# leonsick/s2d

Hardware: AMD Instinct MI355X
Metric: clip-frames/sec fwd+loss, R50 M2F-Video T=8 720p Q=100 (higher is better)
Workload: dtype f32 (f16x3 MFMA for dense contractions); 1 GPU; KDVideoMaskFormer fwd+loss (student+teacher fwd, GT+KD VideoSetCriterion), c4: 2 clips/GPU x T=8 x 720x1280, Q=100, P=160000, N=10 sparse GT instances/clip, encoder dropout 0.3; clips_per_gpu=2, frames_per_clip=8, parallelism=dp1 (clips sharded, no collective), streams=2

## Files before the change

include/s2d_hip.h:

```cpp
#ifndef S2D_HIP_H
#define S2D_HIP_H
#include <stdint.h>

#ifndef HIP_INCLUDE_HIP_HIP_RUNTIME_API_H
typedef struct ihipStream_t *hipStream_t;
#endif

#ifdef __cplusplus
extern "C" {
#endif

#define S2D_OK 0
#define S2D_ERR_ARG (-1)
#define S2D_ERR_LAUNCH (-2)

int s2d_abi_version(void);

int s2d_set_dense_mode(int mode);


int s2d_gemm_nt_f32(const float *A, const float *B, float *C, int M, int N, int K, long lda, long ldb, long ldc,
                    int batch, long strideA, long strideB, long strideC, const float *scale, const float *bias,
                    const float *res, long ldr, long strideR, int res_rows, int res_cols, int relu, const void *B_split,
                    hipStream_t stream);
// ... 6 lines not shown

int s2d_gemm_nt_gate_f32(const float *A, const float *B, float *C, int M, int N, int K, long lda, long ldb, long ldc, const float *scale,
                         const float *res, long ldr, const float *gate, long ldg, float gate_scale, const void *B_split, hipStream_t stream);
int s2d_conv2d_nhwc_gate_f32(const float *x, const float *w, float *y, int N, int H, int W, int Cin, int Cout, int KH, int KW, int stride,
                             int pad, const float *scale, const float *gate, float gate_scale, const void *w_split, hipStream_t stream);
int s2d_gemm_nt_presplit_f32(const void *A_split, const float *B, float *C, int M, int N, int K, long ldb, long ldc, const float *bias,
                             const float *res, long ldr, int res_rows, int res_cols, int relu, const void *B_split, hipStream_t stream);
long s2d_split_weights_words(int N, int K);
long s2d_gemm_rows_launches(void);
int s2d_split_weights_f16(const float *W, int N, int K, long ldw, void *out, hipStream_t stream);

long s2d_ffn_pack_words(int C, int F, int Npost, int pre);
int s2d_ffn_pack_f16(const float *W1, const float *W2, int C, int F, const float *Wpost, int Npost, const float *Wpre, void *out,
                     hipStream_t stream);
int s2d_ffn_fused_f32(const float *x, long M, int C, int F, const void *pack, const float *b1, const float *b2, const float *ln1_gamma,
                      const float *ln1_beta, const float *ln2_gamma, const float *ln2_beta, float eps, float p, uint64_t seed,
                      unsigned site_hidden, unsigned site_out, unsigned row0, float *xn, float *y, int Npost, const float *post_bias,
                      const float *post_pos, int post_S, int post_npos, long post_ldpos, float *post_out, long post_ld,
                      const float *pre_bias, const float *pre_res, unsigned site_pre, hipStream_t stream);

int s2d_conv2d_nhwc_f32(const float *x, const float *w, float *y, int N, int H, int W, int Cin, int Cout, int KH,
                        int KW, int stride, int pad, const float *scale, const float *bias, const float *res,
                        int relu, const void *w_split, hipStream_t stream);

int s2d_gemm_nt_amp_f32(const float *A, const float *B, float *C, int M, int N, int K, long lda, long ldb, long ldc, int batch,
                        long strideA, long strideB, long strideC, const float *scale, const float *bias, const float *res, long ldr,
                        long strideR, int res_rows, int res_cols, int relu, hipStream_t stream);
int s2d_conv2d_nhwc_amp_f32(const float *x, const float *w, float *y, int N, int H, int W, int Cin, int Cout, int KH, int KW, int stride,
                            int pad, const float *scale, const float *bias, const float *res, int relu, hipStream_t stream);


int s2d_msda_forward_f32(const float *value, const int64_t *shapes_host, const int64_t *level_start_host,
                         const float *loc, const float *attn_w, int N, int S, int M, int D, int L, int Lq, int P,
                         float *out, hipStream_t stream);

int s2d_msda_backward_f32(const float *value, const int64_t *shapes_host, const int64_t *level_start_host,
                          const float *loc, const float *attn_w, const float *grad_out, int N, int S, int M, int D,
                          int L, int Lq, int P, float *grad_value, float *grad_loc, float *grad_attn_w,
                          hipStream_t stream);

long s2d_msda_backward_workspace_bytes(const int64_t *shapes_host, int N, int M, int L, int Lq, int P);
int s2d_msda_backward_sorted_f32(const float *value, const int64_t *shapes_host, const int64_t *level_start_host,
                                 const float *loc, const float *attn_w, const float *grad_out, int N, int S, int M, int D,
                                 int L, int Lq, int P, float *grad_value, float *grad_loc, float *grad_attn_w, void *workspace,
                                 long workspace_bytes, hipStream_t stream);
int s2d_msda_backward_sorted_strided_f32(const float *value, long ldv, const int64_t *shapes_host, const int64_t *level_start_host,
// ... 424 lines not shown
```

s2d_amd/csrc/gemm.hip:

```cpp
#include "gemm_epilogue.h"
#include "dropout.h"

namespace {

constexpr int BM = 128, BN = 128, BK = 32, LDS_STRIDE = BK + 4;

template <bool CONV>
__global__ __launch_bounds__(256, 2) void gemm_nt_kernel(GemmParams p)
{
    __shared__ __attribute__((aligned(16))) float lds[2 * (BM + BN) * LDS_STRIDE];
    float *As = lds;
    float *Bs = lds + 2 * BM * LDS_STRIDE;

    const int tid = threadIdx.x, lane = tid & 63, wave = tid >> 6;
    const int wm = wave >> 1, wn = wave & 1;
    const int l32 = lane & 31, h = lane >> 5;

    const int tiles_n = (p.N + BN - 1) / BN, tiles_m = (p.M + BM - 1) / BM;
    const int nwg = tiles_m * tiles_n;
    int bid = blockIdx.x;
    {
        const int q = nwg / 8, r = nwg % 8, xcd = bid % 8, within = bid / 8;
        bid = (xcd < r ? xcd * (q + 1) : r * (q + 1) + (xcd - r) * q) + within;
    }
// ... 205 lines not shown
    q.drop_thresh = thresh;
    q.drop_scale = s2d_dropout_scale(thresh);
    q.drop_k0 = (unsigned)(seed & 0xFFFFFFFFull); q.drop_k1 = (unsigned)(seed >> 32); q.drop_stream = site; q.drop_row0 = row0;
    return launch(q, false, 1, stream);
}

int s2d_conv2d_nhwc_f32(const float *x, const float *w, float *y, int N, int H, int W, int Cin, int Cout, int KH,
                        int KW, int stride, int pad, const float *scale, const float *bias, const float *res,
                        int relu, const void *w_split, hipStream_t stream)
{
    if (Cin & 3) return S2D_ERR_ARG;
    GemmParams p{};
    p.Bsplit = reinterpret_cast<const unsigned int *>(w_split);
    p.Hin = H; p.Win = W; p.Cin = Cin; p.KH = KH; p.KW = KW; p.stride = stride; p.pad = pad;
    p.Hout = (H + 2 * pad - KH) / stride + 1;
    p.Wout = (W + 2 * pad - KW) / stride + 1;
    p.A = x; p.B = w; p.C = y;
    p.M = N * p.Hout * p.Wout; p.N = Cout; p.K = KH * KW * Cin;
    p.lda = 4; p.ldb = p.K; p.ldc = Cout;
    p.scale = scale; p.bias = bias; p.res = res; p.ldr = Cout; p.relu = relu; p.res_cols = Cout;
    return launch(p, true, 1, stream);
}

int s2d_conv2d_nhwc_gate_f32(const float *x, const float *w, float *y, int N, int H, int W, int Cin, int Cout, int KH, int KW, int stride,
                             int pad, const float *scale, const float *gate, float gate_scale, const void *w_split, hipStream_t stream)
{
    if ((Cin & 3) || !gate) return S2D_ERR_ARG;
    GemmParams p{};
    p.Bsplit = reinterpret_cast<const unsigned int *>(w_split);
    p.Hin = H; p.Win = W; p.Cin = Cin; p.KH = KH; p.KW = KW; p.stride = stride; p.pad = pad;
    p.Hout = (H + 2 * pad - KH) / stride + 1;
    p.Wout = (W + 2 * pad - KW) / stride + 1;
    p.A = x; p.B = w; p.C = y;
    p.M = N * p.Hout * p.Wout; p.N = Cout; p.K = KH * KW * Cin;
    p.lda = 4; p.ldb = p.K; p.ldc = Cout;
    p.scale = scale; p.ldr = Cout; p.res_cols = Cout;
    p.gate = gate; p.ldg = Cout; p.gate_scale = gate_scale;
    return launch(p, true, 1, stream);
}

}

extern "C" long s2d_split_weights_words(int N, int K) { return (long)N * ((K + 31) / 32) * 32; }

extern "C" int s2d_split_weights_f16(const float *W, int N, int K, long ldw, void *out, hipStream_t stream)
{
    if (N < 0 || K <= 0 || ldw < K) return S2D_ERR_ARG;
    return s2d_split_weights_launch(W, N, K, ldw, reinterpret_cast<unsigned int *>(out), stream, g_dense_mode == 1);
}

extern "C" int s2d_abi_version(void) { return 11; }

extern "C" int s2d_set_dense_mode(int mode)
{
    if (mode < 0 || mode > 2) return S2D_ERR_ARG;
    g_dense_mode = mode;
    return S2D_OK;
}
```

s2d_amd/csrc/gemm_bf16.hip:

```cpp
#include "gemm_epilogue.h"
#include "gemm_route.h"
#include "dropout.h"
#include <type_traits>

namespace {

typedef __bf16 bf16x2 __attribute__((ext_vector_type(2)));
typedef __bf16 bf16x8 __attribute__((ext_vector_type(8)));

constexpr int BN = GEMM_BN, BK = GEMM_BK, ROWW = 36;

__device__ __forceinline__ void split4_bf16(const f32x4 v, u32x2 &hi, u32x2 &lo)
{
    const f32x2 a = {v[0], v[1]}, b = {v[2], v[3]};
    const bf16x2 ha = __builtin_convertvector(a, bf16x2), hb = __builtin_convertvector(b, bf16x2);
    const unsigned int ua = __builtin_bit_cast(unsigned int, ha), ub = __builtin_bit_cast(unsigned int, hb);
    const f32x2 fa = {__uint_as_float(ua << 16), __uint_as_float(ua & 0xFFFF0000u)};
    const f32x2 fb = {__uint_as_float(ub << 16), __uint_as_float(ub & 0xFFFF0000u)};
    const bf16x2 la = __builtin_convertvector(a - fa, bf16x2), lb = __builtin_convertvector(b - fb, bf16x2);
    hi[0] = ua; hi[1] = ub;
    lo[0] = __builtin_bit_cast(unsigned int, la); lo[1] = __builtin_bit_cast(unsigned int, lb);
}

template <int WM, bool CONV>
// ... 701 lines not shown
            }
        }
        return;
    }
#pragma unroll
    for (int tn = 0; tn < 2; ++tn) {
        const int col = n0 + wn * 64 + tn * 32 + l32;
        if (col >= p.N) continue;
        const float sc = p.scale ? p.scale[col] : 1.f;
        const float bi = p.bias ? p.bias[col] : 0.f;
#pragma unroll
        for (int tm = 0; tm < 2; ++tm) {
#pragma unroll
            for (int r = 0; r < 16; ++r) {
                const int row = mfma32_row(r, h, m0 + wm * 64 + tm * 32);
                if (row >= p.M) continue;
                C[(long)row * p.ldc + col] = scalar_tail(p, res, join(accm[tm][tn][r], accx[tm][tn][r]), sc, bi, row, col);
            }
        }
    }
}

constexpr int HT_H = HALO_PH, HT_W = HALO_PW, HALO_W = HT_W + 2;
template <int PH, int WNW, bool PIPE>
__global__ __launch_bounds__(256, 2) void conv3x3_f16x3_halo_kernel(GemmParams p)
{
    constexpr int HALO_ROWS = (PH + 2) * HALO_W, BNT = 64 * WNW, WROWS = BNT / 32;
    static_assert(PH * HT_W == 64 * (4 / WNW), "four waves of 64 pixels x 64 channels");
    extern __shared__ __attribute__((aligned(16))) unsigned int lds[];
    unsigned int *Ah = lds;
    unsigned int *Bs = lds + HALO_ROWS * ROWW;
    const int tid = threadIdx.x, lane = tid & 63, wave = tid >> 6;
    const int wm = wave / WNW, wn = wave % WNW;
    const int l32 = lane & 31, h = lane >> 5;
    const int H = p.Hin, W = p.Win, Cin = p.Cin;
    const int tiles_x = (W + HT_W - 1) / HT_W, tiles_y = (H + PH - 1) / PH;
    const int tiles_n = (p.N + BNT - 1) / BNT, tiles_m = (p.M / (H * W)) * tiles_y * tiles_x;
    const int nwg = tiles_m * tiles_n;
    int bid = blockIdx.x;
    {
        const int q = nwg / 8, r = nwg % 8, xcd = bid % 8, within = bid / 8;
        bid = (xcd < r ? xcd * (q + 1) : r * (q + 1) + (xcd - r) * q) + within;
    }
    const int tile_m = bid / tiles_n, tile_n = bid % tiles_n;
    const int n0 = tile_n * BNT;
    const int img = tile_m / (tiles_y * tiles_x), trem = tile_m % (tiles_y * tiles_x);
    const int y0 = (trem / tiles_x) * PH, x0 = (trem % tiles_x) * HT_W;

    const __amdgpu_buffer_rsrc_t rsA = __builtin_amdgcn_make_buffer_rsrc(const_cast<float *>(p.A), 0, (int)p.bytesA, 0x00020000);
    const __amdgpu_buffer_rsrc_t rsB = __builtin_amdgcn_make_buffer_rsrc(const_cast<unsigned int *>(p.Bsplit), 0, (int)((long)p.N * p.kblocks * 128L), 0x00020000);
    constexpr int A_IT = (HALO_ROWS * 8 + 255) / 256;
    unsigned int ha_off[A_IT];
    int ha_dst[A_IT];
    bool ha_zero[A_IT];
#pragma unroll
    for (int i = 0; i < A_IT; ++i) {
        const int item = tid + 256 * i;
        const int row = item >> 3, c4 = item & 7;
        const int hy = row / HALO_W, hx = row - hy * HALO_W;
        const int iy = y0 - 1 + hy, ix = x0 - 1 + hx;
        const bool ok = row < HALO_ROWS && iy >= 0 && iy < H && ix >= 0 && ix < W;
        ha_off[i] = ok ? (unsigned int)((((long)img * H + iy) * W + ix) * Cin * 4L + c4 * 16) : 0u;
        ha_zero[i] = !ok;
        ha_dst[i] = row < HALO_ROWS ? row * ROWW + c4 * 2 : -1;
    }
    const int c4 = tid & 7, g = tid >> 3;
    const int r0 = (g & ~7) | ((g & 1) << 2) | ((g >> 1) & 3);
    const int wsel = (c4 & 3) * 4 + (c4 >> 2) * 16;
    unsigned int b_off[WROWS];
#pragma unroll
    for (int i = 0; i < WROWS; ++i) {
        const int n = n0 + r0 + 32 * i;
        b_off[i] = (unsigned int)((long)(n < p.N ? n : p.N - 1) * p.kblocks * 128L + wsel * 4);
    }
    const int cblocks = Cin / 32;
    f32x4 ra[A_IT], rb[WROWS];
    auto load_halo = [&](int cb) {
#pragma unroll
        for (int i = 0; i < A_IT; ++i)
            ra[i] = __builtin_bit_cast(f32x4, __builtin_amdgcn_raw_buffer_load_b128(rsA, (int)(ha_off[i] + (ha_zero[i] ? 0u : (unsigned int)(cb * 128))), 0, 0));
    };
    auto store_halo = [&]() {
#pragma unroll
        for (int i = 0; i < A_IT; ++i) {
            if (ha_dst[i] < 0) continue;
            u32x2 hi, lo;
            split4(ra[i], hi, lo);
            if (ha_zero[i]) { hi = u32x2{0u, 0u}; lo = u32x2{0u, 0u}; }
            *reinterpret_cast<u32x2 *>(Ah + ha_dst[i]) = hi;
            *reinterpret_cast<u32x2 *>(Ah + ha_dst[i] + 16) = lo;
        }
    };
    auto load_w = [&](int tap, int cb) {
        const unsigned int kb = (unsigned int)(tap * cblocks + cb) * 128u;
#pragma unroll
        for (int i = 0; i < WROWS; ++i)
            rb[i] = __builtin_bit_cast(f32x4, __builtin_amdgcn_raw_buffer_load_b128(rsB, (int)b_off[i], (int)kb, 0));
    };
    auto store_w = [&](int buf) {
#pragma unroll
        for (int i = 0; i < WROWS; ++i)
            *reinterpret_cast<f32x4 *>(Bs + (buf * BNT + r0 + 32 * i) * ROWW + wsel) = rb[i];
    };
    int a_row[2];
#pragma unroll
    for (int i = 0; i < 2; ++i) {
        const int pix = wm * 64 + i * 32 + l32;
        a_row[i] = ((pix / HT_W) * HALO_W + (pix % HT_W)) * ROWW + 4 * h;
    }
    f32x16 accm[2][2], accx[2][2];
#pragma unroll
    for (int i = 0; i < 2; ++i)
#pragma unroll
// ... 45 lines not shown
        accx[i][0] = __builtin_amdgcn_mfma_f32_32x32x16_f16(pa[bufi][0], pb[s][0][1], accx[i][0], 0, 0, 0);
        accx[i][1] = __builtin_amdgcn_mfma_f32_32x32x16_f16(pa[bufi][0], pb[s][1][1], accx[i][1], 0, 0, 0);
        accm[i][0] = __builtin_amdgcn_mfma_f32_32x32x16_f16(pa[bufi][0], pb[s][0][0], accm[i][0], 0, 0, 0);
        accm[i][1] = __builtin_amdgcn_mfma_f32_32x32x16_f16(pa[bufi][0], pb[s][1][0], accm[i][1], 0, 0, 0);
    };
    auto compute_pipe = [&](int tap, int buf, int ntap, bool nexta) {
        read_a(1, tap, 0, 1); read_b(buf, 1);
        __builtin_amdgcn_sched_barrier(0);
        group(0, 0, 0);
        __builtin_amdgcn_sched_barrier(0);
        read_a(0, tap, 1, 0);
        __builtin_amdgcn_sched_barrier(0);
        group(1, 0, 1);
        __builtin_amdgcn_sched_barrier(0);
        read_a(1, tap, 1, 1);
        __builtin_amdgcn_sched_barrier(0);
        group(0, 1, 0);
        __builtin_amdgcn_sched_barrier(0);
        if (nexta) read_a(0, ntap, 0, 0);
        __builtin_amdgcn_sched_barrier(0);
        group(1, 1, 1);
        __builtin_amdgcn_sched_barrier(0);
    };
    constexpr bool pipe = PIPE;
    load_halo(0); load_w(0, 0);
    store_halo(); store_w(0);
    __syncthreads();
    const int Q = cblocks * 9;
    int tap = 0, cb = 0;
    if (pipe) { read_a(0, 0, 0, 0); read_b(0, 0); }
    for (int q = 0; q < Q; ++q) {
        const int ntap = tap == 8 ? 0 : tap + 1, ncb = tap == 8 ? cb + 1 : cb;
        if (q + 1 < Q) load_w(ntap, ncb);
        if (tap == 6 && cb + 1 < cblocks) load_halo(cb + 1);
        const bool newhalo = tap == 8 && cb + 1 < cblocks;
        if (pipe) compute_pipe(tap, q & 1, ntap, q + 1 < Q && !newhalo);
        else compute(tap, q & 1);
        if (q + 1 < Q) store_w((q + 1) & 1);
        __syncthreads();
        if (newhalo) { store_halo(); __syncthreads(); }
        if (pipe && q + 1 < Q) {
            if (newhalo) read_a(0, ntap, 0, 0);
            read_b((q + 1) & 1, 0);
        }
        tap = ntap; cb = ncb;
    }

    float *ep = reinterpret_cast<float *>(lds) + wave * 64 * 68;
#pragma unroll
    for (int tm = 0; tm < 2; ++tm)
#pragma unroll
        for (int tn = 0; tn < 2; ++tn)
#pragma unroll
            for (int r = 0; r < 16; ++r)
                ep[mfma32_row(r, h, tm * 32) * 68 + tn * 32 + l32] = join(accm[tm][tn][r], accx[tm][tn][r]);
    const int c4e = lane & 15, rr = lane >> 4;
    const int col = n0 + wn * 64 + c4e * 4;
    if (col < p.N) {
        f32x4 sc = {1.f, 1.f, 1.f, 1.f}, bi = {0.f, 0.f, 0.f, 0.f};
        if (p.scale) sc = *reinterpret_cast<const f32x4 *>(p.scale + col);
        if (p.bias) bi = *reinterpret_cast<const f32x4 *>(p.bias + col);
#pragma unroll 4
        for (int it = 0; it < 16; ++it) {
            const int pix = wm * 64 + it * 4 + rr;
            const int oy = y0 + pix / HT_W, ox = x0 + pix % HT_W;
            if (oy >= H || ox >= W) continue;
            const long row = ((long)img * H + oy) * W + ox;
            f32x4 v = *reinterpret_cast<const f32x4 *>(&ep[(it * 4 + rr) * 68 + c4e * 4]);
// ... 773 lines not shown

int launch_conv7x7s2_stem(const GemmParams &p, int ph, hipStream_t st)
{
    const size_t lds16 = sizeof(float) * 4 * 64 * 68, lds8 = sizeof(float) * 4 * 32 * 68;
    static S2dDevOnce attr_set;
    if (!attr_set.done()) {
        if (hipFuncSetAttribute(reinterpret_cast<const void *>(conv7x7s2_c4_halo_kernel<16>), hipFuncAttributeMaxDynamicSharedMemorySize, (int)lds16) != hipSuccess)
            return S2D_ERR_LAUNCH;
        attr_set.mark();
    }
    const int imgs = p.M / (p.Hout * p.Wout);
    if (ph == 16) hipLaunchKernelGGL(conv7x7s2_c4_halo_kernel<16>, dim3(imgs * cdiv(p.Hout, 16) * cdiv(p.Wout, ST_P)), dim3(256), lds16, st, p);
    else hipLaunchKernelGGL(conv7x7s2_c4_halo_kernel<8>, dim3(imgs * cdiv(p.Hout, 8) * cdiv(p.Wout, ST_P)), dim3(256), lds8, st, p);
    S2D_CHECK_LAUNCH();
    return S2D_OK;
}

int launch_conv3x3_halo(const GemmParams &p, const GemmRoute &r, hipStream_t st)
{
    const size_t lds = sizeof(float) * 4 * 64 * 68;
    static S2dDevOnce attr_set;
    if (!attr_set.done()) {
        for (const void *fn : {reinterpret_cast<const void *>(conv3x3_f16x3_halo_kernel<8, 2, true>), reinterpret_cast<const void *>(conv3x3_f16x3_halo_kernel<16, 1, true>),
                               reinterpret_cast<const void *>(conv3x3_f16x3_halo_kernel<8, 2, false>), reinterpret_cast<const void *>(conv3x3_f16x3_halo_kernel<16, 1, false>)})
            if (hipFuncSetAttribute(fn, hipFuncAttributeMaxDynamicSharedMemorySize, (int)lds) != hipSuccess) return S2D_ERR_LAUNCH;
        attr_set.mark();
    }
    const int imgs = p.M / (p.Hin * p.Win);
    if (r.ph == 16) {
        const int nwg = imgs * cdiv(p.Hin, 16) * cdiv(p.Win, HT_W);
        if (r.pipe) hipLaunchKernelGGL((conv3x3_f16x3_halo_kernel<16, 1, true>), dim3(nwg), dim3(256), lds, st, p);
        else hipLaunchKernelGGL((conv3x3_f16x3_halo_kernel<16, 1, false>), dim3(nwg), dim3(256), lds, st, p);
    } else {
        const int nwg = imgs * cdiv(p.Hin, HT_H) * cdiv(p.Win, HT_W) * cdiv(p.N, BN);
        if (r.pipe) hipLaunchKernelGGL((conv3x3_f16x3_halo_kernel<8, 2, true>), dim3(nwg), dim3(256), lds, st, p);
        else hipLaunchKernelGGL((conv3x3_f16x3_halo_kernel<8, 2, false>), dim3(nwg), dim3(256), lds, st, p);
    }
    S2D_CHECK_LAUNCH();
    return S2D_OK;
}

template <bool CONV, bool BSPLIT>
int launch_w128_v(const GemmParams &p, int batch, hipStream_t st)
{
    const size_t lds = sizeof(float) * 4 * 64 * 68;
    static S2dDevOnce attr_set;
    if (!attr_set.done()) {
        if (hipFuncSetAttribute(reinterpret_cast<const void *>(gemm_bf16x3_w128_kernel<CONV, BSPLIT>),
                                hipFuncAttributeMaxDynamicSharedMemorySize, (int)lds) != hipSuccess)
            return S2D_ERR_LAUNCH;
        attr_set.mark();
    }
    const int nwg = cdiv(p.M, 256) * cdiv(p.N, BN);
    hipLaunchKernelGGL((gemm_bf16x3_w128_kernel<CONV, BSPLIT>), dim3(nwg, batch), dim3(256), lds, st, p);
    S2D_CHECK_LAUNCH();
    return S2D_OK;
}

// ... 28 lines not shown
    const int k = kb * 32 + c4 * 4;
    f32x4 v = {0.f, 0.f, 0.f, 0.f};
    if (vec4) { if (k < K) v = *reinterpret_cast<const f32x4 *>(W + n * ldw + k); }
    else {
        float t[4] = {0.f, 0.f, 0.f, 0.f};
#pragma unroll
        for (int j = 0; j < 4; ++j)
            if (k + j < K) t[j] = W[n * ldw + k + j];
#pragma unroll
        for (int j = 0; j < 4; ++j) {
            float r;
            asm volatile("v_mov_b32 %0, %1" : "=v"(r) : "v"(t[j]));
            v[j] = r;
        }
    }
    u32x2 hi, lo;
    if (BF16) split4_bf16(v, hi, lo);
    else split4(v, hi, lo);
    unsigned int *o = out + nb * 32;
    *reinterpret_cast<u32x2 *>(o + c4 * 2) = hi;
    *reinterpret_cast<u32x2 *>(o + 16 + c4 * 2) = lo;
}

}

int s2d_split_weights_launch(const float *W, int N, int K, long ldw, unsigned int *out, hipStream_t st, int bf16)
{
    const int kblocks = (K + 31) / 32;
    const long n = (long)N * kblocks * 8;
    if (n == 0) return S2D_OK;
    const int vec4 = ((K | ldw) & 3) == 0 && (reinterpret_cast<uintptr_t>(W) & 15) == 0;
    if (bf16) hipLaunchKernelGGL(split_weights_kernel<true>, dim3(cdiv(n, 256)), dim3(256), 0, st, W, N, K, ldw, kblocks, out, vec4);
    else hipLaunchKernelGGL(split_weights_kernel<false>, dim3(cdiv(n, 256)), dim3(256), 0, st, W, N, K, ldw, kblocks, out, vec4);
    S2D_CHECK_LAUNCH();
    return S2D_OK;
}

static GemmSwitches read_gemm_switches()
{
    GemmSwitches s;
    static const int small = s2d_env_int("S2D_GEMM_SMALL", s.small), ws = s2d_env_int("S2D_GEMM_WS", s.ws), hi = s2d_env_int("S2D_GEMM_HI", s.hi),
                     hi_pre = s2d_env_int("S2D_GEMM_HI_PRE", s.hi_pre), pipe = s2d_env_int("S2D_GEMM_PIPE", s.pipe), w128 = s2d_env_int("S2D_GEMM_W128", s.w128),
                     wm = s2d_env_int("S2D_GEMM_WM", s.wm), halo = s2d_env_int("S2D_CONV_HALO", s.halo), halo64 = s2d_env_int("S2D_CONV_HALO64", s.halo64),
                     stem = s2d_env_int("S2D_CONV_STEM", s.stem), stem_ph = s2d_env_int("S2D_CONV_STEM_PH", s.stem_ph);
    s.small = small; s.ws = ws; s.hi = hi; s.hi_pre = hi_pre; s.pipe = pipe; s.w128 = w128; s.wm = wm; s.halo = halo; s.halo64 = halo64; s.stem = stem; s.stem_ph = stem_ph;
    s.rows = s2d_env_int("S2D_GEMM_ROWS", s.rows);
// ... 38 lines not shown
```

s2d_amd/csrc/gemm_params.h:

```cpp
#pragma once

struct GemmParams {
    const float *A, *B;
    float *C;
    int M, N, K;
    long lda, ldb, ldc;
    long sA, sB, sC;
    const float *scale, *bias, *res;
    long ldr, sR;
    int res_rows, res_cols;
    int relu;
    const float *gate;
    long ldg;
    float gate_scale;
    int Hin, Win, Cin, Hout, Wout, KH, KW, stride, pad;
    unsigned int bytesA, bytesB;
    const unsigned int *Bsplit;
    int kblocks;
    const unsigned int *Asplit;
    unsigned int drop_thresh;
    float drop_scale;
    unsigned int drop_k0, drop_k1, drop_stream;
    unsigned int drop_row0;
    const float *zeros, *ones;
};

#ifdef __HIPCC__
struct GemmSwitches;
int s2d_split_weights_launch(const float *W, int N, int K, long ldw, unsigned int *out, hipStream_t st, int bf16);
int s2d_launch_gemm_bf16x3(const GemmParams &p, bool conv, int batch, hipStream_t st, int f16);
int s2d_launch_gemm_small_m(const GemmParams &p, hipStream_t st);
int s2d_launch_gemm_rows(const GemmParams &p, const GemmSwitches &sw, hipStream_t st);
#endif
```

s2d_amd/csrc/gemm_route.h:

```cpp
#pragma once
#include <stdint.h>

#include "gemm_params.h"

constexpr int GEMM_BN = 128, GEMM_BK = 32;
constexpr int HALO_PH = 8, HALO_PW = 16;
constexpr int WS_CONST_N = 16384;

struct GemmSwitches {
    int rows = 1, small = 1, ws = 0, hi = 2, hi_pre = 1, pipe = 1, w128 = 1, wm = 0;
    int halo = 1, halo64 = 1, halo_pipe = 0, stem = 1, stem_ph = 8;
};

enum GemmFamily {
    GEMM_ERR_ARG, GEMM_ROWS, GEMM_SMALL_M, GEMM_F16_WS, GEMM_F16_HI, GEMM_F16, GEMM_CONV3X3_HALO, GEMM_CONV7X7S2_STEM, GEMM_W128, GEMM_T2, GEMM_T4
};

struct GemmRoute {
    GemmFamily family = GEMM_ERR_ARG;
    bool conv = false, bsplit = false, drop = false, res = false, asplit = false;
    bool pipe = false, pre = false;
    int ph = 0;
};

static inline int gemm_cdiv(long a, long b) { return (int)((a + b - 1) / b); }

inline bool s2d_gemm_extents(GemmParams &p, bool conv, int batch)
{
    const long bA = conv ? (long)(p.M / ((long)p.Hout * p.Wout)) * p.Hin * p.Win * p.Cin * 4L : ((long)(p.M - 1) * p.lda + p.K) * 4L;
    const long bB = ((long)(p.N - 1) * p.ldb + p.K) * 4L;
    if (bA > 0xFFFFFF00L || bB > 0xFFFFFF00L) return false;
    p.bytesA = (unsigned int)bA; p.bytesB = (unsigned int)bB;
    if (p.Bsplit) {
        if ((batch > 1 && p.sB != 0) || (long)p.N * ((p.K + 31) / 32) * 128L > 0xFFFFFF00L) return false;
        p.kblocks = (p.K + 31) / 32;
    }
    return true;
}

inline bool s2d_gemm_rows_ok(const GemmParams &p, bool conv, int batch, int f16)
{
    const long bC = ((long)(p.M - 1) * p.ldc + p.N) * 4L, bR = p.res ? ((long)((p.res_rows ? p.res_rows : p.M) - 1) * p.ldr + p.N) * 4L : 0;
    return f16 && !conv && batch == 1 && p.M >= 1 && p.Bsplit && !p.Asplit && !p.gate && !p.drop_thresh && p.K % 32 == 0 && p.K >= 32 && p.K <= 256 &&
           p.N >= 128 && ((p.N | p.ldc | p.ldr | p.res_cols) & 3) == 0 && bC <= 0xFFFFFF00L && bR <= 0xFFFFFF00L;
}

inline bool s2d_gemm_small_m_ok(const GemmParams &p, bool conv, int batch, int f16, const GemmSwitches &sw)
{
    return sw.small && f16 && !conv && batch == 1 && p.M >= 1 && p.M <= 256 && p.Bsplit && !p.Asplit && !p.gate && !p.drop_thresh && p.K >= 64 && p.K % 64 == 0 &&
           (p.lda & 3) == 0 && ((reinterpret_cast<uintptr_t>(p.A) & 15) == 0);
}

inline bool gemm_rows_wins(const GemmParams &p)
{
    if (p.M >= 65536) return (long)p.N * p.K >= 65536;
    return p.M >= 32768 && p.N >= 1024 && p.K >= 256;
}

inline GemmRoute s2d_gemm_route(const GemmParams &p, bool conv, int batch, int f16, const GemmSwitches &sw)
{
    constexpr int BN = GEMM_BN, BK = GEMM_BK;
    GemmRoute r;
    const auto to = [&r](GemmFamily f) { r.family = f; return r; };
    if (!f16 && (p.Asplit || p.gate || p.drop_thresh)) return to(GEMM_ERR_ARG);
    if (sw.rows && s2d_gemm_rows_ok(p, conv, batch, f16) && (sw.rows == 2 || gemm_rows_wins(p))) return to(GEMM_ROWS);
    if (s2d_gemm_small_m_ok(p, conv, batch, f16, sw)) return to(GEMM_SMALL_M);
    r.conv = conv; r.bsplit = p.Bsplit != nullptr; r.drop = p.drop_thresh != 0; r.res = p.res != nullptr;

    const long bC = ((long)(p.M - 1) * p.ldc + p.N) * 4L, bR = p.res ? ((long)((p.res_rows ? p.res_rows : p.M) - 1) * p.ldr + p.N) * 4L : 0;
    const bool ws_ok = sw.ws && f16 && batch == 1 && !p.gate && p.N <= WS_CONST_N && (conv || !p.scale) && p.K >= 7 * BK - (BK - 1) && ((p.N | p.ldc | p.ldr | p.res_cols) & 3) == 0 &&
                       (conv ? (p.Cin % 4 == 0 && (p.Bsplit || p.K % BK == 0)) : p.K % BK == 0) &&
                       bC <= 0xFFFFFF00L && bR <= 0xFFFFFF00L && (!p.res_rows || p.res_rows >= 64) &&
                       (!p.drop_thresh || (((p.N | p.ldc) & 7) == 0 && (!p.res || ((p.ldr | p.res_cols) & 7) == 0)));
    if (p.Asplit) {
        const bool ok = f16 && !conv && batch == 1 && p.Bsplit && !p.scale && p.N <= WS_CONST_N && p.K >= 7 * BK - (BK - 1) && p.K % BK == 0 &&
                        ((p.N | p.ldc | p.ldr | p.res_cols) & 3) == 0 && bC <= 0xFFFFFF00L && bR <= 0xFFFFFF00L &&
                        (long)p.M * p.kblocks * 128L <= 0xFFFFFF00L && (!p.res_rows || p.res_rows >= 64) &&
                        (!p.drop_thresh || (((p.N | p.ldc) & 7) == 0 && (!p.res || ((p.ldr | p.res_cols) & 7) == 0)));
        if (!ok) return to(GEMM_ERR_ARG);
        r.asplit = true;
        return to(GEMM_F16_WS);
    }
    if (ws_ok && !conv && (sw.ws == 2 || (p.Bsplit && (long)gemm_cdiv(p.M, 128) * gemm_cdiv(p.N, BN) >= 512))) return to(GEMM_F16_WS);
    if (ws_ok && conv && !p.drop_thresh && (sw.ws == 2 || (long)gemm_cdiv(p.M, 128) * gemm_cdiv(p.N, BN) >= 512)) return to(GEMM_F16_WS);
    if (p.gate && (!f16 || batch != 1 || p.drop_thresh || ((p.N | p.ldc | p.ldr | p.res_cols | p.ldg) & 3))) return to(GEMM_ERR_ARG);
    if (p.drop_thresh) {
        if (!f16 || conv || ((p.N | p.ldc) & 7) || (p.res && (((p.ldr | p.res_cols) & 7)))) return to(GEMM_ERR_ARG);
        r.pipe = true;
        return to(GEMM_F16);
    }
    if (f16) {
        if (sw.stem && conv && p.KH == 7 && p.KW == 7 && p.stride == 2 && p.pad == 3 && p.Cin == 4 && p.N <= 64 && p.N > 32 && p.Bsplit && batch == 1 &&
            ((p.N | p.ldc | p.ldr) & 3) == 0 && !p.res_rows && p.res_cols == p.N && !p.gate && (long)p.Hin * p.Win * 16L * (p.M / ((long)p.Hout * p.Wout)) < 0x7fffffffL) {
            r.ph = sw.stem_ph == 16 ? 16 : 8;
            return to(GEMM_CONV7X7S2_STEM);
        }
        const int ph = p.N <= 64 ? 16 : HALO_PH;
        if (sw.halo && conv && p.KH == 3 && p.KW == 3 && p.stride == 1 && p.pad == 1 && p.Cin % 32 == 0 && p.Bsplit && batch == 1 && (p.N > 64 || (sw.halo64 && p.N > 32)) &&
            ((p.N | p.ldc | p.ldr) & 3) == 0 && !p.res_rows && p.res_cols == p.N && !p.gate &&
            (sw.halo == 2 || (long)p.Hin * p.Win * 100 >= (long)gemm_cdiv(p.Hin, ph) * ph * gemm_cdiv(p.Win, HALO_PW) * HALO_PW * 88)) {
            r.ph = ph;
            r.pipe = sw.halo_pipe != 0;
            return to(GEMM_CONV3X3_HALO);
        }
        bool use_hi;
        if (sw.hi != 2) use_hi = sw.hi == 1;
        else if (conv && p.KH > 1) use_hi = p.N <= 64;
        else if (p.N <= 64 || p.K <= 128 || !p.Bsplit) use_hi = true;
        else if (p.K >= 512) use_hi = false;
        else {
            const float w128 = (float)(gemm_cdiv(p.N, 128) * 128) / p.N, w64 = (float)(gemm_cdiv(p.N, 64) * 64) / p.N;
            use_hi = w128 > w64 + 0.1f;
        }
        if (use_hi) {
            r.pre = sw.hi_pre && p.Bsplit && p.res && !p.gate && p.K <= 4 * BK && ((p.N | p.ldc | p.ldr | p.res_cols) & 3) == 0;
            return to(GEMM_F16_HI);
        }
        r.pipe = sw.pipe != 0;
        return to(GEMM_F16);
    }
    if (sw.w128 && !conv && (long)gemm_cdiv(p.M, 256) * gemm_cdiv(p.N, BN) * batch >= (sw.w128 == 2 ? 1 : 512)) return to(GEMM_W128);
    bool big = (long)gemm_cdiv(p.M, 256) * gemm_cdiv(p.N, BN) * batch >= 256;
    if (sw.wm == 2) big = false;
    if (sw.wm == 4) big = true;
    return to(big ? GEMM_T4 : GEMM_T2);
// ... 2 lines not shown
```

s2d_amd/ops.py:

```python
import torch

from ._lib import lib
from .weight_cache import DerivedCache, bump_version, clear_weight_cache, mark_static, owner_of, repack, version_of


PROFILE = None


def _stream():
    return torch.cuda.current_stream().cuda_stream


class _Ev:
    __slots__ = ("h",)

    def __init__(self):
        self.h = lib().call("s2d_prof_event_create")
        if not self.h:
            raise RuntimeError("hipEventCreateWithFlags failed")

    def record(self):
        lib().call("s2d_prof_event_record", self.h, _stream())

    def elapsed_time(self, other):
# ... 30 lines not shown
    if t is None:
        return
    if not t.is_cuda or not t.is_contiguous() or t.dtype != dtype:
        raise RuntimeError(f"s2d op needs a contiguous {dtype} CUDA tensor, got {t.dtype} {t.device} contiguous={t.is_contiguous()}")


_MODE = "f16x3"
_SPLIT = DerivedCache()


def _static_split(B, N, K, ldb):
    if _MODE == "f32" or N * ((K + 31) // 32) * 128 > 0xFFFFFF00:
        return None
    base = owner_of(B)
    if not (isinstance(base, torch.nn.Parameter) or getattr(base, "_s2d_static", False) or getattr(B, "_s2d_static", False)):
        return None

    def split(img):
        lib().call("s2d_split_weights_f16", B, N, K, ldb, img, _stream())
        return img

    return _SPLIT.get((B.data_ptr(), N, K, ldb, _MODE), (base,),
                      lambda: split(torch.empty((lib().call("s2d_split_weights_words", N, K),), device=B.device, dtype=torch.int32)), split)


def set_dense_mode(mode):
    global _MODE
    lib().call("s2d_set_dense_mode", {"f32": 0, "bf16x3": 1, "f16x3": 2}[mode])
    _MODE = mode


_AMP = [0]


class amp_fp16:

    def __init__(self, enabled=True):
        self.enabled = bool(enabled)

    def __enter__(self):
        _AMP[0] += 1 if self.enabled else 0

    def __exit__(self, *a):
        _AMP[0] -= 1 if self.enabled else 0


# ... 175 lines not shown
    return y


dropout = dropout_apply


_DROP_CALLS = [0]


def next_dropout_seed():
    _DROP_CALLS[0] += 1
    return (torch.initial_seed() * 0x9E3779B97F4A7C15 + _DROP_CALLS[0] * 0xD1B54A32D192ED03) & 0xFFFFFFFFFFFFFFFF


def conv2d_nhwc(x, w, stride=1, pad=0, scale=None, bias=None, res=None, relu=False):
    for t in (x, w, scale, bias, res):
        _chk(t)
    N, H, W, Cin = x.shape
    Cout, KH, KW, _ = w.shape
    Ho = (H + 2 * pad - KH) // stride + 1
    Wo = (W + 2 * pad - KW) // stride + 1
    y = torch.empty((N, Ho, Wo, Cout), device=x.device, dtype=torch.float32)
    ws = None if amp_active() else _static_split(w, Cout, KH * KW * Cin, KH * KW * Cin)
    with _Timed(2.0 * N * Ho * Wo * Cout * KH * KW * (3 if Cin == 4 else Cin),
                ("conv", KH, N * Ho * Wo, Cout, KH * KW * Cin, 4.0 * (x.numel() + w.numel() + N * Ho * Wo * Cout * (2 if res is not None else 1)))):
        if amp_active():
            lib().call("s2d_conv2d_nhwc_amp_f32", x, w, y, N, H, W, Cin, Cout, KH, KW, stride, pad, scale, bias, res, int(relu), _stream())
            return y
        lib().call("s2d_conv2d_nhwc_f32", x, w, y, N, H, W, Cin, Cout, KH, KW, stride, pad, scale, bias, res, int(relu), ws,
                   _stream())
    return y


import numpy as _np


def _host_i64(a):
    if isinstance(a, torch.Tensor):
        a = a.detach().cpu().numpy()
    return _np.ascontiguousarray(a, dtype=_np.int64)


def msda_forward(value, shapes, level_start, loc, attn_w):
    for t in (value, loc, attn_w):
        _chk(t)
    N, S, M, D = value.shape
    Lq, L, P = loc.shape[1], loc.shape[3], loc.shape[4]
    sh, ls = _host_i64(shapes), _host_i64(level_start)
    out = torch.empty((N, Lq, M * D), device=value.device, dtype=torch.float32)
    lib().call("s2d_msda_forward_f32", value, sh, ls, loc, attn_w, N, S, M, D, L, Lq, P, out, _stream())
    return out

# ... 416 lines not shown
```

Measured before the change: 179.1 clip-frames/s.

## Stream prepacked MFMA weight fragments directly in 3x3 halo conv kernel

```diff
diff --git a/include/s2d_hip.h b/include/s2d_hip.h
--- a/include/s2d_hip.h
+++ b/include/s2d_hip.h
@@ -52,6 +52,12 @@
 int s2d_conv2d_nhwc_f32(const float *x, const float *w, float *y, int N, int H, int W, int Cin, int Cout, int KH,
                         int KW, int stride, int pad, const float *scale, const float *bias, const float *res,
                         int relu, const void *w_split, hipStream_t stream);
+long s2d_conv3x3_frag_words(int Cout, int Cin);
+long s2d_conv3x3_direct_wins(long M, int Cout, int Cin);
+int s2d_conv3x3_frag_weights_f16(const float *w, int Cout, int Cin, void *out, hipStream_t stream);
+int s2d_conv2d_nhwc_frag_f32(const float *x, const float *w, float *y, int N, int H, int W, int Cin, int Cout, int KH,
+                             int KW, int stride, int pad, const float *scale, const float *bias, const float *res,
+                             int relu, const void *w_split, const void *w_frag, hipStream_t stream);
 
 int s2d_gemm_nt_amp_f32(const float *A, const float *B, float *C, int M, int N, int K, long lda, long ldb, long ldc, int batch,
                         long strideA, long strideB, long strideC, const float *scale, const float *bias, const float *res, long ldr,
diff --git a/s2d_amd/csrc/gemm.hip b/s2d_amd/csrc/gemm.hip
--- a/s2d_amd/csrc/gemm.hip
+++ b/s2d_amd/csrc/gemm.hip
@@ -1,4 +1,5 @@
 #include "gemm_epilogue.h"
+#include "gemm_route.h"
 #include "dropout.h"
 
 namespace {
@@ -251,6 +252,25 @@
     return launch(p, true, 1, stream);
 }
 
+int s2d_conv2d_nhwc_frag_f32(const float *x, const float *w, float *y, int N, int H, int W, int Cin, int Cout, int KH,
+                             int KW, int stride, int pad, const float *scale, const float *bias, const float *res,
+                             int relu, const void *w_split, const void *w_frag, hipStream_t stream)
+{
+    if (Cin & 3) return S2D_ERR_ARG;
+    if (w_frag && (!w_split || KH != 3 || KW != 3 || stride != 1 || pad != 1 || (Cin & 31) || g_dense_mode != 2)) return S2D_ERR_ARG;
+    GemmParams p{};
+    p.Bsplit = reinterpret_cast<const unsigned int *>(w_split);
+    p.Bfrag = reinterpret_cast<const unsigned int *>(w_frag);
+    p.Hin = H; p.Win = W; p.Cin = Cin; p.KH = KH; p.KW = KW; p.stride = stride; p.pad = pad;
+    p.Hout = (H + 2 * pad - KH) / stride + 1;
+    p.Wout = (W + 2 * pad - KW) / stride + 1;
+    p.A = x; p.B = w; p.C = y;
+    p.M = N * p.Hout * p.Wout; p.N = Cout; p.K = KH * KW * Cin;
+    p.lda = 4; p.ldb = p.K; p.ldc = Cout;
+    p.scale = scale; p.bias = bias; p.res = res; p.ldr = Cout; p.relu = relu; p.res_cols = Cout;
+    return launch(p, true, 1, stream);
+}
+
 int s2d_conv2d_nhwc_gate_f32(const float *x, const float *w, float *y, int N, int H, int W, int Cin, int Cout, int KH, int KW, int stride,
                              int pad, const float *scale, const float *gate, float gate_scale, const void *w_split, hipStream_t stream)
 {
@@ -278,6 +298,16 @@
     return s2d_split_weights_launch(W, N, K, ldw, reinterpret_cast<unsigned int *>(out), stream, g_dense_mode == 1);
 }
 
+extern "C" long s2d_conv3x3_frag_words(int Cout, int Cin) { return Cout > 0 && Cin > 0 && Cin % 32 == 0 ? conv3x3_frag_words(Cout, Cin) : 0; }
+
+extern "C" long s2d_conv3x3_direct_wins(long M, int Cout, int Cin) { return conv3x3_direct_wins(M, Cout, Cin) ? 1 : 0; }
+
+extern "C" int s2d_conv3x3_frag_weights_f16(const float *w, int Cout, int Cin, void *out, hipStream_t stream)
+{
+    if (Cout <= 0 || Cin <= 0 || Cin % 32 || g_dense_mode != 2 || conv3x3_frag_words(Cout, Cin) * 4L > 0x7FFFFF00L) return S2D_ERR_ARG;
+    return s2d_conv3x3_frag_weights_launch(w, Cout, Cin, reinterpret_cast<unsigned int *>(out), stream);
+}
+
 extern "C" int s2d_abi_version(void) { return 11; }
 
 extern "C" int s2d_set_dense_mode(int mode)
diff --git a/s2d_amd/csrc/gemm_bf16.hip b/s2d_amd/csrc/gemm_bf16.hip
--- a/s2d_amd/csrc/gemm_bf16.hip
+++ b/s2d_amd/csrc/gemm_bf16.hip
@@ -747,11 +747,14 @@
 }
 
 constexpr int HT_H = HALO_PH, HT_W = HALO_PW, HALO_W = HT_W + 2;
-template <int PH, int WNW, bool PIPE>
+constexpr int conv3x3_halo_buffers(int ph) { return 2 * 2 * (ph + 2) * HALO_W * ROWW * 4 <= 160 * 1024 ? 2 : 1; }
+template <int PH, int WNW, bool PIPE, bool DIRECT = false>
 __global__ __launch_bounds__(256, 2) void conv3x3_f16x3_halo_kernel(GemmParams p)
 {
     constexpr int HALO_ROWS = (PH + 2) * HALO_W, BNT = 64 * WNW, WROWS = BNT / 32;
     static_assert(PH * HT_W == 64 * (4 / WNW), "four waves of 64 pixels x 64 channels");
+    static_assert(!(PIPE && DIRECT), "the fragment pipeline is a form of the LDS-weight loop");
+    constexpr int HB = conv3x3_halo_buffers(PH);
     extern __shared__ __attribute__((aligned(16))) unsigned int lds[];
     unsigned int *Ah = lds;
     unsigned int *Bs = lds + HALO_ROWS * ROWW;
@@ -775,19 +778,23 @@
     const __amdgpu_buffer_rsrc_t rsA = __builtin_amdgcn_make_buffer_rsrc(const_cast<float *>(p.A), 0, (int)p.bytesA, 0x00020000);
     const __amdgpu_buffer_rsrc_t rsB = __builtin_amdgcn_make_buffer_rsrc(const_cast<unsigned int *>(p.Bsplit), 0, (int)((long)p.N * p.kblocks * 128L), 0x00020000);
     constexpr int A_IT = (HALO_ROWS * 8 + 255) / 256;
-    unsigned int ha_off[A_IT];
-    int ha_dst[A_IT];
-    bool ha_zero[A_IT];
-#pragma unroll
-    for (int i = 0; i < A_IT; ++i) {
-        const int item = tid + 256 * i;
+    auto halo_item = [&](int t, int i, unsigned int &off, bool &zero, int &dst) {
+        const int item = t + 256 * i;
         const int row = item >> 3, c4 = item & 7;
         const int hy = row / HALO_W, hx = row - hy * HALO_W;
         const int iy = y0 - 1 + hy, ix = x0 - 1 + hx;
         const bool ok = row < HALO_ROWS && iy >= 0 && iy < H && ix >= 0 && ix < W;
-        ha_off[i] = ok ? (unsigned int)((((long)img * H + iy) * W + ix) * Cin * 4L + c4 * 16) : 0u;
-        ha_zero[i] = !ok;
-        ha_dst[i] = row < HALO_ROWS ? row * ROWW + c4 * 2 : -1;
+        off = ok ? (unsigned int)((((long)img * H + iy) * W + ix) * Cin * 4L + c4 * 16) : 0u;
+        zero = !ok;
+        dst = row < HALO_ROWS ? row * ROWW + c4 * 2 : -1;
+    };
+    constexpr int A_KEEP = DIRECT ? 1 : A_IT;
+    unsigned int ha_off[A_KEEP];
+    int ha_dst[A_KEEP];
+    bool ha_zero[A_KEEP];
+    if constexpr (!DIRECT) {
+#pragma unroll
+        for (int i = 0; i < A_IT; ++i) halo_item(tid, i, ha_off[i], ha_zero[i], ha_dst[i]);
     }
     const int c4 = tid & 7, g = tid >> 3;
     const int r0 = (g & ~7) | ((g & 1) << 2) | ((g >> 1) & 3);
@@ -801,19 +808,31 @@
     const int cblocks = Cin / 32;
     f32x4 ra[A_IT], rb[WROWS];
     auto load_halo = [&](int cb) {
-#pragma unroll
-        for (int i = 0; i < A_IT; ++i)
-            ra[i] = __builtin_bit_cast(f32x4, __builtin_amdgcn_raw_buffer_load_b128(rsA, (int)(ha_off[i] + (ha_zero[i] ? 0u : (unsigned int)(cb * 128))), 0, 0));
-    };
-    auto store_halo = [&]() {
+        int t = tid;
+        if constexpr (DIRECT) asm volatile("" : "+v"(t));
 #pragma unroll
         for (int i = 0; i < A_IT; ++i) {
-            if (ha_dst[i] < 0) continue;
+            unsigned int off; bool zero; int dst;
+            if constexpr (DIRECT) halo_item(t, i, off, zero, dst);
+            else { off = ha_off[i]; zero = ha_zero[i]; }
+            ra[i] = __builtin_bit_cast(f32x4, __builtin_amdgcn_raw_buffer_load_b128(rsA, (int)(off + (zero ? 0u : (unsigned int)(cb * 128))), 0, 0));
+        }
+    };
+    auto store_halo = [&](int hbuf = 0) {
+        unsigned int *ah = Ah + hbuf * (HALO_ROWS * ROWW);
+        int t = tid;
+        if constexpr (DIRECT) asm volatile("" : "+v"(t));
+#pragma unroll
+        for (int i = 0; i < A_IT; ++i) {
+            unsigned int off; bool zero; int dst;
+            if constexpr (DIRECT) halo_item(t, i, off, zero, dst);
+            else { zero = ha_zero[i]; dst = ha_dst[i]; }
+            if (dst < 0) continue;
             u32x2 hi, lo;
             split4(ra[i], hi, lo);
-            if (ha_zero[i]) { hi = u32x2{0u, 0u}; lo = u32x2{0u, 0u}; }
-            *reinterpret_cast<u32x2 *>(Ah + ha_dst[i]) = hi;
-            *reinterpret_cast<u32x2 *>(Ah + ha_dst[i] + 16) = lo;
+            if (zero) { hi = u32x2{0u, 0u}; lo = u32x2{0u, 0u}; }
+            *reinterpret_cast<u32x2 *>(ah + dst) = hi;
+            *reinterpret_cast<u32x2 *>(ah + dst + 16) = lo;
         }
     };
     auto load_w = [&](int tap, int cb) {
@@ -905,6 +924,63 @@
         group(1, 1, 1);
         __builtin_amdgcn_sched_barrier(0);
     };
+    if constexpr (DIRECT) {
+        const int NT = 4 * ((p.N + 127) / 128);
+        const __amdgpu_buffer_rsrc_t rsF = __builtin_amdgcn_make_buffer_rsrc(const_cast<unsigned int *>(p.Bfrag), 0, (int)((long)p.kblocks * NT * 4096L), 0x00020000);
+        const unsigned int f_off = (unsigned int)(((n0 + wn * 64) >> 5) * 4096 + lane * 16);
+        f16x8 fb[2][2][2][2];
+        auto load_f = [&](int set, int tap, int cb) {
+            const unsigned int kb = (unsigned int)(tap * cblocks + cb) * (unsigned int)NT * 4096u;
+#pragma unroll
+            for (int t2 = 0; t2 < 2; ++t2)
+#pragma unroll
+                for (int s = 0; s < 2; ++s)
+#pragma unroll
+                    for (int hl = 0; hl < 2; ++hl)
+                        fb[set][s][t2][hl] = __builtin_bit_cast(f16x8, __builtin_amdgcn_raw_buffer_load_b128(rsF, (int)(f_off + (unsigned int)((t2 * 4 + s * 2 + hl) * 1024)), (int)kb, 0));
+        };
+        auto compute_d = [&](int set, int tap, int hbuf) {
+            const unsigned int *ah_ = Ah + hbuf * (HALO_ROWS * ROWW) + ((tap / 3) * HALO_W + (tap % 3)) * ROWW;
+#pragma unroll
+            for (int s = 0; s < 2; ++s) {
+#pragma unroll
+                for (int i = 0; i < 2; ++i) {
+                    const f16x8 ah = *reinterpret_cast<const f16x8 *>(ah_ + a_row[i] + 8 * s);
+                    const f16x8 al = *reinterpret_cast<const f16x8 *>(ah_ + a_row[i] + 16 + 8 * s);
+                    accx[i][0] = __builtin_amdgcn_mfma_f32_32x32x16_f16(al, fb[set][s][0][0], accx[i][0], 0, 0, 0);
+                    accx[i][1] = __builtin_amdgcn_mfma_f32_32x32x16_f16(al, fb[set][s][1][0], accx[i][1], 0, 0, 0);
+                    accx[i][0] = __builtin_amdgcn_mfma_f32_32x32x16_f16(ah, fb[set][s][0][1], accx[i][0], 0, 0, 0);
+                    accx[i][1] = __builtin_amdgcn_mfma_f32_32x32x16_f16(ah, fb[set][s][1][1], accx[i][1], 0, 0, 0);
+                    accm[i][0] = __builtin_amdgcn_mfma_f32_32x32x16_f16(ah, fb[set][s][0][0], accm[i][0], 0, 0, 0);
+                    accm[i][1] = __builtin_amdgcn_mfma_f32_32x32x16_f16(ah, fb[set][s][1][0], accm[i][1], 0, 0, 0);
+                }
+            }
+        };
+        load_halo(0); load_f(0, 0, 0);
+        store_halo(0);
+        __syncthreads();
+        for (int cb0 = 0; cb0 < cblocks; cb0 += 2) {
+#pragma unroll
+            for (int par = 0; par < 2; ++par) {
+                const int cb = cb0 + par;
+                if (cb >= cblocks) break;
+                const bool more = cb + 1 < cblocks;
+                const int hbuf = HB == 2 ? par : 0;
+#pragma unroll
+                for (int tap = 0; tap < 9; ++tap) {
+                    const int set = (par + tap) & 1;
+                    if (tap < 8) load_f(set ^ 1, tap + 1, cb);
+                    else if (more && HB == 2) load_f(set ^ 1, 0, cb + 1);
+                    if (tap == (HB == 2 ? 2 : 8) && more) load_halo(cb + 1);
+                    if (HB == 2 && tap == 6 && more) store_halo(hbuf ^ 1);
+                    compute_d(set, tap, hbuf);
+                }
+                if (HB == 2) { if (more) __syncthreads(); }
+                else if (more) { __syncthreads(); store_halo(0); load_f(par ^ 1, 0, cb + 1); __syncthreads(); }
+            }
+        }
+        __syncthreads();
+    } else {
     constexpr bool pipe = PIPE;
     load_halo(0); load_w(0, 0);
     store_halo(); store_w(0);
@@ -927,6 +1003,7 @@
             read_b((q + 1) & 1, 0);
         }
         tap = ntap; cb = ncb;
+    }
     }
 
     float *ep = reinterpret_cast<float *>(lds) + wave * 64 * 68;
@@ -1746,18 +1823,23 @@
     static S2dDevOnce attr_set;
     if (!attr_set.done()) {
         for (const void *fn : {reinterpret_cast<const void *>(conv3x3_f16x3_halo_kernel<8, 2, true>), reinterpret_cast<const void *>(conv3x3_f16x3_halo_kernel<16, 1, true>),
-                               reinterpret_cast<const void *>(conv3x3_f16x3_halo_kernel<8, 2, false>), reinterpret_cast<const void *>(conv3x3_f16x3_halo_kernel<16, 1, false>)})
+                               reinterpret_cast<const void *>(conv3x3_f16x3_halo_kernel<8, 2, false>), reinterpret_cast<const void *>(conv3x3_f16x3_halo_kernel<16, 1, false>),
+                               reinterpret_cast<const void *>(conv3x3_f16x3_halo_kernel<8, 2, false, true>), reinterpret_cast<const void *>(conv3x3_f16x3_halo_kernel<16, 1, false, true>)})
             if (hipFuncSetAttribute(fn, hipFuncAttributeMaxDynamicSharedMemorySize, (int)lds) != hipSuccess) return S2D_ERR_LAUNCH;
         attr_set.mark();
     }
+    static_assert(sizeof(unsigned int) * conv3x3_halo_buffers(8) * 10 * HALO_W * ROWW <= sizeof(float) * 4 * 64 * 68 && sizeof(unsigned int) * conv3x3_halo_buffers(16) * 18 * HALO_W * ROWW <= sizeof(float) * 4 * 64 * 68, "halo buffers fit the epilogue staging");
+    if (r.direct && (long)conv3x3_frag_words(p.N, p.Cin) * 4L > 0x7FFFFF00L) return S2D_ERR_ARG;
     const int imgs = p.M / (p.Hin * p.Win);
     if (r.ph == 16) {
         const int nwg = imgs * cdiv(p.Hin, 16) * cdiv(p.Win, HT_W);
         if (r.pipe) hipLaunchKernelGGL((conv3x3_f16x3_halo_kernel<16, 1, true>), dim3(nwg), dim3(256), lds, st, p);
+        else if (r.direct) hipLaunchKernelGGL((conv3x3_f16x3_halo_kernel<16, 1, false, true>), dim3(nwg), dim3(256), lds, st, p);
         else hipLaunchKernelGGL((conv3x3_f16x3_halo_kernel<16, 1, false>), dim3(nwg), dim3(256), lds, st, p);
     } else {
         const int nwg = imgs * cdiv(p.Hin, HT_H) * cdiv(p.Win, HT_W) * cdiv(p.N, BN);
         if (r.pipe) hipLaunchKernelGGL((conv3x3_f16x3_halo_kernel<8, 2, true>), dim3(nwg), dim3(256), lds, st, p);
+        else if (r.direct) hipLaunchKernelGGL((conv3x3_f16x3_halo_kernel<8, 2, false, true>), dim3(nwg), dim3(256), lds, st, p);
         else hipLaunchKernelGGL((conv3x3_f16x3_halo_kernel<8, 2, false>), dim3(nwg), dim3(256), lds, st, p);
     }
     S2D_CHECK_LAUNCH();
@@ -1832,6 +1914,34 @@
     *reinterpret_cast<u32x2 *>(o + 16 + c4 * 2) = lo;
 }
 
+__global__ __launch_bounds__(256) void conv3x3_frag_weights_kernel(const float *__restrict__ W, int N, int K, int kblocks, int NT, unsigned int *__restrict__ out)
+{
+    const long i = (long)blockIdx.x * 256 + threadIdx.x;
+    if (i >= (long)NT * 32 * kblocks * 8) return;
+    const int c4 = (int)(i & 7);
+    const long nb = i >> 3;
+    const int kb = (int)(nb % kblocks);
+    const int n = (int)(nb / kblocks);
+    f32x4 v = {0.f, 0.f, 0.f, 0.f};
+    if (n < N) v = *reinterpret_cast<const f32x4 *>(W + (long)n * K + kb * 32 + c4 * 4);
+    u32x2 hi, lo;
+    split4(v, hi, lo);
+    const int s = c4 >> 2, h = (c4 >> 1) & 1, j = (c4 & 1) * 2;
+    unsigned int *o = out + (((long)kb * NT + (n >> 5)) * 4 + s * 2) * 256 + (h * 32 + (n & 31)) * 4 + j;
+    *reinterpret_cast<u32x2 *>(o) = hi;
+    *reinterpret_cast<u32x2 *>(o + 256) = lo;
+}
+
+}
+
+int s2d_conv3x3_frag_weights_launch(const float *W, int Cout, int Cin, unsigned int *out, hipStream_t st)
+{
+    const int kblocks = 9 * (Cin / 32), NT = 4 * cdiv(Cout, 128);
+    const long n = (long)NT * 32 * kblocks * 8;
+    if (n == 0) return S2D_OK;
+    hipLaunchKernelGGL(conv3x3_frag_weights_kernel, dim3(cdiv(n, 256)), dim3(256), 0, st, W, Cout, 9 * Cin, kblocks, NT, out);
+    S2D_CHECK_LAUNCH();
+    return S2D_OK;
 }
 
 int s2d_split_weights_launch(const float *W, int N, int K, long ldw, unsigned int *out, hipStream_t st, int bf16)
diff --git a/s2d_amd/csrc/gemm_params.h b/s2d_amd/csrc/gemm_params.h
--- a/s2d_amd/csrc/gemm_params.h
+++ b/s2d_amd/csrc/gemm_params.h
@@ -23,11 +23,13 @@
     unsigned int drop_k0, drop_k1, drop_stream;
     unsigned int drop_row0;
     const float *zeros, *ones;
+    const unsigned int *Bfrag;
 };
 
 #ifdef __HIPCC__
 struct GemmSwitches;
 int s2d_split_weights_launch(const float *W, int N, int K, long ldw, unsigned int *out, hipStream_t st, int bf16);
+int s2d_conv3x3_frag_weights_launch(const float *W, int Cout, int Cin, unsigned int *out, hipStream_t st);
 int s2d_launch_gemm_bf16x3(const GemmParams &p, bool conv, int batch, hipStream_t st, int f16);
 int s2d_launch_gemm_small_m(const GemmParams &p, hipStream_t st);
 int s2d_launch_gemm_rows(const GemmParams &p, const GemmSwitches &sw, hipStream_t st);
diff --git a/s2d_amd/csrc/gemm_route.h b/s2d_amd/csrc/gemm_route.h
--- a/s2d_amd/csrc/gemm_route.h
+++ b/s2d_amd/csrc/gemm_route.h
@@ -21,6 +21,7 @@
     bool conv = false, bsplit = false, drop = false, res = false, asplit = false;
     bool pipe = false, pre = false;
     int ph = 0;
+    bool direct = false;
 };
 
 static inline int gemm_cdiv(long a, long b) { return (int)((a + b - 1) / b); }
@@ -55,6 +56,14 @@
 {
     if (p.M >= 65536) return (long)p.N * p.K >= 65536;
     return p.M >= 32768 && p.N >= 1024 && p.K >= 256;
+}
+
+inline long conv3x3_frag_words(int Cout, int Cin) { return (long)(9 * (Cin / 32)) * (4 * gemm_cdiv(Cout, 128)) * 1024L; }
+
+inline bool conv3x3_direct_wins(long M, int Cout, int Cin)
+{
+    (void)M; (void)Cin;
+    return Cout > 64;
 }
 
 inline GemmRoute s2d_gemm_route(const GemmParams &p, bool conv, int batch, int f16, const GemmSwitches &sw)
@@ -101,6 +110,7 @@
             (sw.halo == 2 || (long)p.Hin * p.Win * 100 >= (long)gemm_cdiv(p.Hin, ph) * ph * gemm_cdiv(p.Win, HALO_PW) * HALO_PW * 88)) {
             r.ph = ph;
             r.pipe = sw.halo_pipe != 0;
+            r.direct = !r.pipe && p.Bfrag;
             return to(GEMM_CONV3X3_HALO);
         }
         bool use_hi;
diff --git a/s2d_amd/ops.py b/s2d_amd/ops.py
--- a/s2d_amd/ops.py
+++ b/s2d_amd/ops.py
@@ -76,6 +76,24 @@
 
     return _SPLIT.get((B.data_ptr(), N, K, ldb, _MODE), (base,),
                       lambda: split(torch.empty((lib().call("s2d_split_weights_words", N, K),), device=B.device, dtype=torch.int32)), split)
+
+
+_FRAG = DerivedCache()
+
+
+def _static_frag(w, M, Cout, Cin, force=False):
+    if _MODE != "f16x3" or Cin % 32 or not (force or lib().call("s2d_conv3x3_direct_wins", M, Cout, Cin)):
+        return None
+    base = owner_of(w)
+    if not (isinstance(base, torch.nn.Parameter) or getattr(base, "_s2d_static", False) or getattr(w, "_s2d_static", False)):
+        return None
+
+    def frag(img):
+        lib().call("s2d_conv3x3_frag_weights_f16", w, Cout, Cin, img, _stream())
+        return img
+
+    return _FRAG.get((w.data_ptr(), Cout, Cin), (base,),
+                     lambda: frag(torch.empty((lib().call("s2d_conv3x3_frag_words", Cout, Cin),), device=w.device, dtype=torch.int32)), frag)
 
 
 def set_dense_mode(mode):
@@ -297,12 +315,13 @@
     Wo = (W + 2 * pad - KW) // stride + 1
     y = torch.empty((N, Ho, Wo, Cout), device=x.device, dtype=torch.float32)
     ws = None if amp_active() else _static_split(w, Cout, KH * KW * Cin, KH * KW * Cin)
+    wf = _static_frag(w, N * Ho * Wo, Cout, Cin) if ws is not None and (KH, KW, stride, pad) == (3, 3, 1, 1) and Cout > 32 else None
     with _Timed(2.0 * N * Ho * Wo * Cout * KH * KW * (3 if Cin == 4 else Cin),
                 ("conv", KH, N * Ho * Wo, Cout, KH * KW * Cin, 4.0 * (x.numel() + w.numel() + N * Ho * Wo * Cout * (2 if res is not None else 1)))):
         if amp_active():
             lib().call("s2d_conv2d_nhwc_amp_f32", x, w, y, N, H, W, Cin, Cout, KH, KW, stride, pad, scale, bias, res, int(relu), _stream())
             return y
-        lib().call("s2d_conv2d_nhwc_f32", x, w, y, N, H, W, Cin, Cout, KH, KW, stride, pad, scale, bias, res, int(relu), ws,
+        lib().call("s2d_conv2d_nhwc_frag_f32", x, w, y, N, H, W, Cin, Cout, KH, KW, stride, pad, scale, bias, res, int(relu), ws, wf,
                    _stream())
     return y
 
```

Result: no change. 178.8 clip-frames/s (-0.2%).
